# seongq/flowmse

Hardware: AMD Instinct MI355X
Metric: enhanced spectrogram-frames/sec at N=5 solver steps (higher is better)
Workload: dtype f32; 1 GPU; BASELINE config[1]: batch=8 synthetic complex spectrograms [8,1,256,256] per GPU, N=5 euler steps (5 NFE), NCSN++ (65.6M params, synthetic weights), precision mode fp32; global_batch=8, frames=256, solver_steps=5, parallelism=dp1 (per-utterance, final RCCL gather only), launch_mode=eager launches of the per-shape launch list (the library's default), hip_graph_launches=0, finite_output_checked=True

## Files before the change

flowmse_amd/csrc/common.h:

```cpp
#pragma once
#include <hip/hip_runtime.h>
#include <stdint.h>

namespace flowse {

enum { OK = 0, ERR_ARG = 1, ERR_HIP = 2, ERR_STATE = 3, ERR_SHAPE = 4 };

void set_error(const char* fmt, ...);
int hip_fail(hipError_t e, const char* what, const char* file, int line);

#define FLOWSE_HIP(call)                                                        \
    do {                                                                        \
        hipError_t _e = (call);                                                 \
        if (_e != hipSuccess) return ::flowse::hip_fail(_e, #call, __FILE__, __LINE__); \
    } while (0)

#define FLOWSE_LAUNCH_CHECK()                                                   \
    do {                                                                        \
        hipError_t _e = hipGetLastError();                                      \
        if (_e != hipSuccess) return ::flowse::hip_fail(_e, "kernel launch", __FILE__, __LINE__); \
    } while (0)

enum { DT_F32 = 0, DT_BF16 = 1, DT_F16 = 2 };
struct bf16_t { unsigned short v; };
// ... 61 lines not shown
    }
    static __device__ __forceinline__ float4 rnd4(float4 v) {
        return make_float4((float)(_Float16)v.x, (float)(_Float16)v.y, (float)(_Float16)v.z, (float)(_Float16)v.w);
    }
    static __device__ __forceinline__ float ld1(const f16_t* p) { return (float)__builtin_bit_cast(_Float16, p->v); }
    static __device__ __forceinline__ void st1(f16_t* p, float v) {
        const _Float16 x = (_Float16)v;
        p->v = __builtin_bit_cast(unsigned short, x);
    }
};
template <class ST> struct Vec16 { static constexpr int N = 16 / (int)sizeof(ST); };
template <class ST>
__device__ __forceinline__ void ld16(const ST* p, float* v) {
    if constexpr (sizeof(ST) == 4) {
        const float4 t = *reinterpret_cast<const float4*>(p);
        v[0] = t.x; v[1] = t.y; v[2] = t.z; v[3] = t.w;
    } else {
        const uint4 t = *reinterpret_cast<const uint4*>(p);
        const unsigned w[4] = {t.x, t.y, t.z, t.w};
#pragma unroll
        for (int i = 0; i < 4; ++i) {
            if constexpr (St<ST>::dt == DT_BF16) {
                v[2 * i] = __uint_as_float(w[i] << 16);
                v[2 * i + 1] = __uint_as_float(w[i] & 0xffff0000u);
            } else {
                v[2 * i] = (float)__builtin_bit_cast(_Float16, (unsigned short)(w[i] & 0xffffu));
                v[2 * i + 1] = (float)__builtin_bit_cast(_Float16, (unsigned short)(w[i] >> 16));
            }
        }
    }
}
template <class ST>
__device__ __forceinline__ void st16_round(ST* p, float* v) {
    if constexpr (sizeof(ST) == 4) {
        *reinterpret_cast<float4*>(p) = make_float4(v[0], v[1], v[2], v[3]);
    } else {
        unsigned w[4];
#pragma unroll
        for (int i = 0; i < 4; ++i) {
            if constexpr (St<ST>::dt == DT_BF16) {
                w[i] = St<bf16_t>::pack2(v[2 * i], v[2 * i + 1]);
                v[2 * i] = __uint_as_float(w[i] << 16);
                v[2 * i + 1] = __uint_as_float(w[i] & 0xffff0000u);
            } else {
                const _Float16 a = (_Float16)v[2 * i], b = (_Float16)v[2 * i + 1];
                w[i] = (unsigned)__builtin_bit_cast(unsigned short, a) | ((unsigned)__builtin_bit_cast(unsigned short, b) << 16);
                v[2 * i] = (float)a;
                v[2 * i + 1] = (float)b;
            }
        }
        *reinterpret_cast<uint4*>(p) = make_uint4(w[0], w[1], w[2], w[3]);
    }
}
#define FLOWSE_DT_SWITCH(dt, ST, ...)                                          \
    switch (dt) {                                                              \
        case ::flowse::DT_F32: { using ST = float; __VA_ARGS__; } break;       \
        case ::flowse::DT_BF16: { using ST = ::flowse::bf16_t; __VA_ARGS__; } break; \
        default: { using ST = ::flowse::f16_t; __VA_ARGS__; } break;           \
    }

struct GnParams {
    const float* mean;
    const float* scale;
    const float* beta;
};

struct Stat4 {
    float4 p, s1, s2;
    int n;
    __device__ __forceinline__ void init() {
        n = 0;
        p = s1 = s2 = make_float4(0.f, 0.f, 0.f, 0.f);
    }
    __device__ __forceinline__ void add(const float4& v) {
        if (n == 0) p = v;
        const float dx = v.x - p.x, dy = v.y - p.y, dz = v.z - p.z, dw = v.w - p.w;
        s1.x += dx; s1.y += dy; s1.z += dz; s1.w += dw;
        s2.x = fmaf(dx, dx, s2.x); s2.y = fmaf(dy, dy, s2.y); s2.z = fmaf(dz, dz, s2.z); s2.w = fmaf(dw, dw, s2.w);
        ++n;
    }
    __device__ __forceinline__ void finish(float* out8) const {
        const float inv = n > 0 ? 1.f / (float)n : 0.f;
        const float a[4] = {s1.x, s1.y, s1.z, s1.w}, q[4] = {s2.x, s2.y, s2.z, s2.w}, pv[4] = {p.x, p.y, p.z, p.w};
#pragma unroll
        for (int j = 0; j < 4; ++j) {
            out8[j] = pv[j] + a[j] * inv;
            out8[4 + j] = fmaxf(q[j] - a[j] * a[j] * inv, 0.f);
        }
    }
};
__device__ __forceinline__ void chan_merge4(float& nA, float* acc8, float nB, const float* in8) {
    if (nB <= 0.f) return;
    const float n = nA + nB, w = nB / n;
#pragma unroll
    for (int j = 0; j < 4; ++j) {
        const float d = in8[j] - acc8[j];
        acc8[j] += d * w;
        acc8[4 + j] += in8[4 + j] + d * d * nA * w;
    }
    nA = n;
}

struct ConvArgs {
    const float* in1;
    const float* in2;
    int C1, C2;
    const float* w;
    const float* bias;
    const float* bias2;
    int bias2_stride;
    const float* res;
    float* out;
    int B, H, W, Cout;
    int taps;
    float scale;
    int ksplit = 1;
    float* partial = nullptr;
    const float* partial2 = nullptr;
    int ksplit2 = 0;
    const float* bias_x = nullptr;
    float* stats = nullptr;
    int stats_nblk = 0;
    GnParams gn = {nullptr, nullptr, nullptr};
    int gn_silu = 0;
    const void* wq = nullptr;
    int terms = 0;
    int wq_f16 = 0;
    const void* wfrag = nullptr;
    const void* sc1 = nullptr;
    const void* sc2 = nullptr;
    int SC1 = 0, SC2 = 0;
    const void* wfrag_sc = nullptr;
    const float* wino = nullptr;
    const float* wino2 = nullptr;
    const float* wsm = nullptr;
    const float* wsm16 = nullptr;
    int in_dt = DT_F32, out_dt = DT_F32;
};
int conv16_ksplit(int B, int H, int W, int Cin, int Cout, int taps);
bool conv16_uses_halo(int B, int H, int W, int C1, int C2, int Cout, int taps);
void pc16_set_channel_blocks(int mode);
bool conv16_uses_pc(int B, int H, int W, int C1, int C2, int Cout, int taps);
int conv16_stats_blocks(int B, int H, int W, int Cin, int Cout, int taps);
int launch_convert(const void* src, int src_dt, void* dst, int dst_dt, int64_t n, hipStream_t s);
int launch_f43_weights(const float* w_packed, int Cout, int Cin, float* out, hipStream_t s);
int launch_pc16_weights(const void* w16, int Cout, int Cin, void* dst, hipStream_t s, int taps = 9);
bool conv16_smallm_ok(int B, int H, int W, int C1, int C2, int Cout, int taps);
int conv16_smallm_stats_blocks(int B, int H, int W);
inline int64_t conv_wino_numel(int Cout, int Cin) { return (int64_t)Cout * 18 * Cin; }
int launch_w2d_weights(const float* w_packed, int Cout, int Cin, float* out, hipStream_t s);
inline int64_t conv_w2d_numel(int Cout, int Cin) { return (int64_t)Cout * 24 * Cin; }
bool conv_w2d_shape_ok(int B, int H, int W, int C1, int C2, int Cout, int taps);
bool conv_supports_w2d(int B, int H, int W, int C1, int C2, int Cout, int taps);
bool conv_smallm_ok(int B, int H, int W, int C1, int C2, int Cout, int taps);
int launch_smallm_weights(const float* w_packed, int Cout, int taps, int Cin, float* out, hipStream_t s, bool tile16 = false);
bool conv_smallm_tile16(int B, int H, int W);
int conv_smallm_stats_blocks(int B, int H, int W);
bool conv1x1_stream_ok(int B, int H, int W, int C1, int C2, int Cout, int taps);
int conv1x1_stream_stats_blocks(int B, int H, int W);
bool conv_w2d_enabled();
bool conv_supports_wino(int B, int H, int W, int C1, int C2, int Cout, int taps);
bool conv_f43_wide(int B, int H, int W, int Cout);
void pack_conv_bf16(const float* w, int Cout, int Cin, int terms, uint16_t* dst, bool f16 = false);
inline int64_t conv_bf16_numel(int Cout, int Cin, int terms) { return (int64_t)Cout * 9 * Cin * (terms == 1 ? 1 : 2); }
bool conv_supports_bf16(int B, int H, int W, int C1, int C2, int Cout, int taps);
bool conv_supports_fused_gn(int B, int H, int W, int C1, int C2, int Cout, int taps);
bool conv_supports_head4(int B, int H, int W, int C1, int C2, int Cout, int taps);
int conv_fused_stats_blocks(int B, int H, int W, int Cin, int Cout, int taps);
int launch_conv(const ConvArgs& a, hipStream_t s, bool with_reduce = true);
int launch_splitk_reduce(const ConvArgs& a, hipStream_t s);
void conv_note_route(const char* a, const char* b = "", const char* c = "");
const char* conv_last_route();
bool conv_reduce_gn_ok(int B, int HW, int Cout);
int launch_splitk_reduce_gn(const ConvArgs& a, const float* gamma, const float* beta, float eps, int silu, int apply,
                            float* gn_mean, float* gn_scale, hipStream_t s);
int conv_ksplit(int B, int H, int W, int Cin, int Cout, int taps);
int conv_splitk_stats_group(int HW);
bool conv_splitk_is_wino(int B, int H, int W, int Cin, int Cout, int taps);
bool conv_cin4_uses_mfma(int B, int H, int W, int Cout, int taps);
int conv_cin4_stats_blocks(int B, int H, int W, int Cout);

int launch_conv_cin4(const ConvArgs& a, hipStream_t s);

int gn_partial_blocks(int HW, int C);
int gn_pixels_per_block(int HW, int nblk);
int launch_gn_stats(const void* in1, int C1, const void* in2, int C2, int B, int HW,
                    float* partial , int nblk, hipStream_t s, int dt = DT_F32);
int launch_gn_finalize(const float* partial1, int nblk1, int C1, const float* partial2, int nblk2, int C2, int B,
                       int HW, int G, const float* gamma, float eps, float* mean ,
                       float* scale , hipStream_t s);

int launch_gn_finalize_apply(const void* in1, const float* partial1, int nblk1, int C1, const void* in2,
                             const float* partial2, int nblk2, int C2, int B, int HW, int G, const float* gamma,
                             const float* beta, float eps, int silu, void* out, hipStream_t s, int in_dt = DT_F32,
                             int out_dt = DT_F32);
int launch_gn_apply(const void* in1, int C1, const void* in2, int C2, int B, int HW,
                    GnParams gn, int silu, void* out, hipStream_t s, int in_dt = DT_F32, int out_dt = DT_F32);

int launch_fir_down(const void* in, int B, int H, int W, int C, GnParams gn, int silu, void* out,
                    hipStream_t s, void* out2 = nullptr, int dt = DT_F32);
int launch_fir_up(const void* in, int B, int H, int W, int C, GnParams gn, int silu, const void* add,
                  void* out, hipStream_t s, void* out2 = nullptr, int dt = DT_F32);
int launch_upfirdn2d_nchw(const float* in, const float* kernel, int planes, int in_h, int in_w, int kh,
                          int kw, int up_x, int up_y, int down_x, int down_y, int pad_x0, int pad_x1,
                          int pad_y0, int pad_y1, float* out, int out_h, int out_w, hipStream_t s);

int launch_attention(const void* qkv, int B, int L, int C, void* out, hipStream_t s, int dt = DT_F32);

struct CallBlock {
    const float* x;
    const float* y;
    const float* t;
    float* out;
    int mode;
    float dt;
    const float* x0 = nullptr;
    const float* acc_in = nullptr;
    float* acc_out = nullptr;
    float a = 0.f, b = 0.f;
};
int launch_set_call(CallBlock* d_cb, const CallBlock& value, hipStream_t s);
int launch_fill_times(float* d_ts, const float* ts, int N, int B, hipStream_t s);
int launch_pack_input(const float* x_c64, const float* y_c64, int B, int F, int T, float* out4, hipStream_t s,
                      const CallBlock* cb = nullptr);
int launch_gfp(const float* t, const float* Wf, int B, int E, float* out, hipStream_t s, const CallBlock* cb = nullptr);
int launch_linear(const float* in, int B, int K, const float* W, const float* bias, int R, int act,
                  float* out, int out_stride, hipStream_t s);
int launch_head(const float* pyr4, const float* t, const float* Wout , const float* bout ,
                int B, int F, int T, int mode, const float* x_c64, float dt, float* out_c64, hipStream_t s,
                const CallBlock* cb = nullptr);
int launch_stft_compress(const float* sig, int B, int L, float scale_in, float* out_c64, int T, int Tpad, float factor,
                         float exponent, hipStream_t s);
int launch_istft_decompress(const float* spec_c64, int B, int T, int Tpad, float factor, float exponent, float* out,
                            int Lout, float scale_out, hipStream_t s);
int launch_stft_compress_chunks(const float* sig, int L, float scale_in, float* out_c64, int K, int Tc, int hop,
                                float factor, float exponent, hipStream_t s);
int launch_istft_decompress_chunks(const float* chunks_c64, int K, int Tc, int hop, float factor, float exponent,
                                   float* out, int Lout, float scale_out, hipStream_t s);
int launch_axpy(const float* y, const float* z, float sigma, int64_t n, float* out, hipStream_t s);
int launch_keyed_noise(const float* y, const uint64_t* keys, const int32_t* frame0, uint64_t seed, float sigma, float* out,
                       int B, int F, int T, hipStream_t s);

}
```

flowmse_amd/csrc/conv_w2d.hip:

```cpp
#include "conv_common.h"

#ifdef FLOWSE_MEASURE_W2D
namespace flowse { __device__ unsigned long long g_w2d_ts[256 * 64]; }
extern "C" int flowse_debug_w2d_ts(unsigned long long* host, int n) {
    return hipMemcpyFromSymbol(host, HIP_SYMBOL(flowse::g_w2d_ts), (size_t)n * 8) == hipSuccess ? 0 : 1;
}
#ifdef FLOWSE_MEASURE_W2D_WAVES
#define W2_TS(K) if ((threadIdx.x & 63) == 0 && blockIdx.x < 256 && (K) >= 4 && ((K) - 4) % 3 == 0 && ((K) - 4) / 3 < 8) \
        flowse::g_w2d_ts[blockIdx.x * 64 + (threadIdx.x >> 6) * 8 + ((K) - 4) / 3] = __builtin_amdgcn_s_memrealtime();
#else
#define W2_TS(K) if (threadIdx.x == 0 && blockIdx.x < 256 && (K) < 64) flowse::g_w2d_ts[blockIdx.x * 64 + (K)] = __builtin_amdgcn_s_memrealtime();
#endif
#else
#define W2_TS(K)
#endif

namespace flowse {

constexpr int W2_HROW = 18 * LDS_ROW + 8;
constexpr int W2_HBUF = 18 * W2_HROW;
constexpr int W2_XDEST = 4 * 3 * 256;

struct W2Tile {
    int y0, x0;
    unsigned hin;
    unsigned woff;
};

template <int CH, int NJ>
__device__ __forceinline__ void w2d_out(f32x16 (&acc)[3][NJ], float* X, int b, int y0, int x0, int n0) {
    const ConvArgs* ap = (const ConvArgs*)__builtin_amdgcn_kernarg_segment_ptr();
    asm volatile("" : "+s"(ap));
    const ConvArgs& a = *ap;
    const int tid = threadIdx.x;
    int lane = tid & 63;
    asm volatile("" : "+v"(lane));
    const int wave = __builtin_amdgcn_readfirstlane(tid >> 6);
    const int hq = wave & 3;
    const int jD = wave >> 2, gD = wave & 3;
    const bool dest = jD < NJ;
    const int li = lane & 31, kh = lane >> 5;
    const int W = a.W, Cout = a.Cout;
    const int ch0 = n0 + jD * 32;
    const int pl = lane >> 3, cq = lane & 7;
    const bool has_res = a.res != nullptr;
    const int64_t pix0 = ((int64_t)b * a.H + y0 + 4 * gD) * W + x0;
    const float* resb = a.res + pix0 * Cout + ch0 + cq * 4;
    float* outb = a.out + pix0 * Cout + ch0 + cq * 4;
    int roff[8];
#pragma unroll
    for (int i = 0; i < 8; ++i) {
        const int pp = i * 8 + pl;
        roff[i] = ((pp >> 4) * W + (pp & 15)) * Cout;
    }
    float4 rres[8];
    if (has_res && dest) {
#pragma unroll
        for (int i = 0; i < 8; ++i) rres[i] = *reinterpret_cast<const float4*>(resb + roff[i]);
    }
    float* Xd = X + wave * W2_XDEST;
    auto give = [&]() {
#pragma unroll
        for (int D = 0; D < 4 * NJ; ++D) {
            const int jd = D >> 2, gd = D & 3;
            float4 v0, v1, v2;
            float* e0 = &v0.x; float* e1 = &v1.x; float* e2 = &v2.x;
#pragma unroll
            for (int e = 0; e < 4; ++e) {
                const int r = 4 * gd + e;
                const float s12 = acc[1][jd][r] + acc[2][jd][r];
                if (CH == 0) {
                    e0[e] = acc[0][jd][r] + s12;
                    e1[e] = acc[1][jd][r] - acc[2][jd][r];
                    e2[e] = s12;
                } else {
                    e0[e] = s12;
                    e1[e] = acc[1][jd][r] - acc[2][jd][r];
                    e2[e] = acc[0][jd][r];
                }
            }
            float* dst = X + D * W2_XDEST + (hq * 3) * 256 + lane * 4;
            *reinterpret_cast<float4*>(dst) = v0;
            *reinterpret_cast<float4*>(dst + 256) = v1;
            *reinterpret_cast<float4*>(dst + 512) = v2;
        }
    };
    auto take = [&](float (&S)[2][3][4]) {
#pragma unroll
        for (int s = 0; s < 4; ++s) {
#pragma unroll
            for (int c = 0; c < 3; ++c) {
                const float4 t = *reinterpret_cast<const float4*>(Xd + (s * 3 + c) * 256 + lane * 4);
                const float* q = &t.x;
#pragma unroll
                for (int e = 0; e < 4; ++e) {
                    if (s == 0) S[0][c][e] = q[e];
                    if (s == 1) { S[0][c][e] += q[e]; S[1][c][e] = q[e]; }
                    if (s == 2) { S[0][c][e] += q[e]; S[1][c][e] -= q[e]; }
                    if (s == 3) S[1][c][e] -= q[e];
                }
            }
        }
    };
    float SA[2][3][4], SB[2][3][4];
    if (CH == 0) give();
    __syncthreads();
    if (dest) take(SA);
    __syncthreads();
    if (CH == 1) give();
    __syncthreads();
    if (!dest) return;
    float4 bq = make_float4(0.f, 0.f, 0.f, 0.f), bq2 = bq;
    if (a.bias) bq = *reinterpret_cast<const float4*>(a.bias + ch0 + cq * 4);
    if (a.bias2) bq2 = *reinterpret_cast<const float4*>(a.bias2 + (int64_t)b * a.bias2_stride + ch0 + cq * 4);
    take(SB);
    float* T = Xd;
    __builtin_amdgcn_wave_barrier();
#pragma unroll
    for (int x = 0; x < 2; ++x)
#pragma unroll
        for (int e = 0; e < 4; ++e) {
            const float A = SA[x][0][e], Bv = SA[x][1][e], Cv = SA[x][2][e];
            const float D = SB[x][0][e], E = SB[x][1][e], Fv = SB[x][2][e];
            const float o0 = A + D, o1 = fmaf(2.f, E, Bv), o2 = fmaf(4.f, D, Cv), o3 = fmaf(8.f, E, Bv) + Fv;
            const int col = 2 * (e + 4 * kh) + x;
            T[(0 * 16 + col) * 32 + li] = o0;
            T[(1 * 16 + col) * 32 + li] = o1;
            T[(2 * 16 + col) * 32 + li] = o2;
            T[(3 * 16 + col) * 32 + li] = o3;
        }
    __builtin_amdgcn_wave_barrier();
    bq.x += bq2.x; bq.y += bq2.y; bq.z += bq2.z; bq.w += bq2.w;
    const float scale = a.scale;
    float4 piv = make_float4(0.f, 0.f, 0.f, 0.f), s1 = piv, s2 = piv;
#pragma unroll
    for (int i = 0; i < 8; ++i) {
        const int pp = i * 8 + pl;
        float4 v = *reinterpret_cast<const float4*>(T + pp * 32 + cq * 4);
        v.x += bq.x; v.y += bq.y; v.z += bq.z; v.w += bq.w;
        if (has_res) { v.x += rres[i].x; v.y += rres[i].y; v.z += rres[i].z; v.w += rres[i].w; }
        v.x *= scale; v.y *= scale; v.z *= scale; v.w *= scale;
        *reinterpret_cast<float4*>(outb + roff[i]) = v;
        if (i == 0) piv = v;
        const float dx = v.x - piv.x, dy = v.y - piv.y, dz = v.z - piv.z, dw = v.w - piv.w;
        s1.x += dx; s1.y += dy; s1.z += dz; s1.w += dw;
        s2.x = fmaf(dx, dx, s2.x); s2.y = fmaf(dy, dy, s2.y); s2.z = fmaf(dz, dz, s2.z); s2.w = fmaf(dw, dw, s2.w);
    }
    if (!a.stats) return;
    float mean[4] = {piv.x + s1.x * 0.125f, piv.y + s1.y * 0.125f, piv.z + s1.z * 0.125f, piv.w + s1.w * 0.125f};
    float m2[4] = {fmaxf(s2.x - s1.x * s1.x * 0.125f, 0.f), fmaxf(s2.y - s1.y * s1.y * 0.125f, 0.f),
                   fmaxf(s2.z - s1.z * s1.z * 0.125f, 0.f), fmaxf(s2.w - s1.w * s1.w * 0.125f, 0.f)};
    float cnt = 8.f;
#pragma unroll
    for (int off = 8; off < 64; off <<= 1) {
#pragma unroll
        for (int j = 0; j < 4; ++j) {
            const float mo = __shfl_xor(mean[j], off), qo = __shfl_xor(m2[j], off);
            const float d = mo - mean[j];
            m2[j] = m2[j] + qo + d * d * (0.5f * cnt);
            mean[j] = 0.5f * (mean[j] + mo);
        }
        cnt *= 2.f;
    }
    if (pl == 0) {
        const int strip = ((y0 >> 2) + gD) * (W >> 4) + (x0 >> 4);
        float* dst = a.stats + (((int64_t)b * a.stats_nblk + strip) * Cout + ch0 + cq * 4) * 2;
        *reinterpret_cast<float4*>(dst) = make_float4(mean[0], m2[0], mean[1], m2[1]);
        *reinterpret_cast<float4*>(dst + 4) = make_float4(mean[2], m2[2], mean[3], m2[3]);
    }
}

template <int GN, int CH, int NJ>
__device__ __forceinline__ void conv3x3_w2d_body(const ConvArgs& a, float* smem, int tpb) {
    constexpr int BN = 32 * NJ;
    constexpr int H_LOADS = 6;
    float* Hs = smem;

    const int tid = threadIdx.x;
    W2_TS(0)
    const int H = a.H, W = a.W, HW = H * W;
    const int C1 = a.C1, C2 = a.C2, Cin = C1 + C2;
    const int n_ntiles = a.Cout / BN;
    const int bid = xcd_remap(blockIdx.x, gridDim.x);
    const int mg = bid / n_ntiles;
    const int nt = bid - mg * n_ntiles;
    const int tiles_x = W >> 4, tiles_img = tiles_x * (H >> 4);
    const int n0 = nt * BN;
    const int wave = __builtin_amdgcn_readfirstlane(tid >> 6);
    const int col4 = tid & 7, slot = tid >> 3;
    const bool s_on = slot < 54;
    const int s_hx = slot >= 36 ? 2 : slot >= 18 ? 1 : 0, s_hy = slot - 18 * s_hx;
    const unsigned s_pix = (unsigned)(s_hy * W + s_hx);
    const int s_lds = s_hy * W2_HROW + s_hx * LDS_ROW + 4 * (col4 ^ ((s_hy >> 2) & 1));
    int s_st = s_lds + W2_HBUF;
    int dflip = W2_HBUF;
    const int bsmp = (mg * tpb) / tiles_img;
    const int b = bsmp;
    const int64_t sbase = (int64_t)bsmp * HW - W - 1;
    const int spix = HW + 2 * W + 2;
    const __amdgpu_buffer_rsrc_t rsrc1 =
        __builtin_amdgcn_make_buffer_rsrc(const_cast<float*>(a.in1 + sbase * C1), 0, spix * C1 * 4, 0x00020000);
    const __amdgpu_buffer_rsrc_t rsrc2 = __builtin_amdgcn_make_buffer_rsrc(
        const_cast<float*>(C2 ? a.in2 + sbase * C2 : a.in1), 0, C2 ? spix * C2 * 4 : 0, 0x00020000);
    auto make_tile = [&](int mt) {
        W2Tile t;
        const int tt = mt - bsmp * tiles_img;
        int ty, tx;
        if ((tiles_x & 3) == 0) {
            const int per_strip = 4 * (H >> 4);
            const int strip = tt / per_strip, w = tt - strip * per_strip;
            ty = w >> 2;
            tx = strip * 4 + (w & 3);
        } else {
            ty = tt / tiles_x;
            tx = tt - ty * tiles_x;
        }
        t.y0 = ty * 16;
        t.x0 = tx * 16;
        const bool rowin = s_on && (unsigned)(t.y0 - 1 + s_hy) < (unsigned)H;
        t.hin = 0;
#pragma unroll
        for (int q = 0; q < H_LOADS; ++q)
            t.hin |= (rowin && (unsigned)(t.x0 - 1 + s_hx + 3 * q) < (unsigned)W) ? (1u << q) : 0u;
        t.woff = (unsigned)(t.y0 * W + t.x0);
        return t;
    };
    const W2Tile first = make_tile(mg * tpb);
    int cur_y0 = first.y0, cur_x0 = first.x0;
    const __amdgpu_buffer_rsrc_t rsrcw =
        __builtin_amdgcn_make_buffer_rsrc(const_cast<float*>(a.wino2), 0, a.Cout * 24 * Cin * 4, 0x00020000);

    u32x4 rh[3];
    float4 g_mu, g_sc, g_be;
    unsigned st_hin = first.hin;

    auto hload = [&](const W2Tile& t, int chunk, int Q) -> u32x4 {
        const int c0 = chunk * KC;
        const bool second = c0 >= C1;
        const unsigned cs = (unsigned)(second ? C2 : C1);
        const unsigned soff = ((t.woff + 3u * (unsigned)Q) * cs + (unsigned)(second ? c0 - C1 : c0)) * 4u;
        const unsigned off = ((t.hin >> Q) & 1u) ? (s_pix * cs + (unsigned)col4 * 4u) * 4u : OOB;
        return second ? __builtin_amdgcn_raw_buffer_load_b128(rsrc2, off, soff, 0)
                      : __builtin_amdgcn_raw_buffer_load_b128(rsrc1, off, soff, 0);
    };
    auto gparams = [&](int chunk, unsigned hin) {
        if (GN) {
            const int cg = chunk * KC + col4 * 4;
            const float rowf = (hin >> 1) & 1u ? 1.f : 0.f;
            g_mu = *reinterpret_cast<const float4*>(a.gn.mean + (int64_t)b * Cin + cg);
            g_sc = *reinterpret_cast<const float4*>(a.gn.scale + (int64_t)b * Cin + cg);
            g_be = *reinterpret_cast<const float4*>(a.gn.beta + cg);
            g_sc.x *= rowf; g_sc.y *= rowf; g_sc.z *= rowf; g_sc.w *= rowf;
            g_be.x *= rowf; g_be.y *= rowf; g_be.z *= rowf; g_be.w *= rowf;
        }
    };
    auto gloadH = [&](const W2Tile& t, int chunk, int h) {
#pragma unroll
        for (int q = 0; q < 3; ++q) rh[q] = hload(t, chunk, 3 * h + q);
        if (h == 0) {
            gparams(chunk, t.hin);
            st_hin = t.hin;
        }
    };
    auto xform1 = [&](int Q) {
        if (GN) rh[Q % 3] = gn_quad<GN>(rh[Q % 3], g_mu, g_sc, g_be, (Q == 0 || Q == 5) ? ((st_hin >> Q) & 1u) != 0 : true);
    };
    auto lstoreH = [&](int h) {
        float* Hb = Hs + s_st + 9 * h * LDS_ROW;
        if (s_on) {
#pragma unroll
            for (int q = 0; q < 3; ++q) *reinterpret_cast<u32x4*>(Hb + 3 * q * LDS_ROW) = rh[q];
        }
    };

    const int lane = tid & 63;
    const int hq = wave & 3;
    const int li = lane & 31, kh = lane >> 5;
    const int ur = li >> 3, uc = li & 7;
    const int ca = hq == 0 ? 0 : hq == 2 ? 2 : 1, cb = hq == 2 ? 1 : hq == 3 ? 3 : 2;
    f32x2 sg2 = {hq == 1 ? 1.f : -1.f, hq == 1 ? 1.f : -1.f};
    asm volatile("" : "+v"(sg2));
    const int base = (4 * ur + CH) * W2_HROW + 2 * uc * LDS_ROW;
    const int k0 = 4 * (kh ^ (ur & 1)), k1 = 4 * (kh ^ (ur & 1) ^ 1);
    int aA0 = base + ca * LDS_ROW + k0, aA1 = base + ca * LDS_ROW + k1;
    int aB0 = base + cb * LDS_ROW + k0, aB1 = base + cb * LDS_ROW + k1;

    const int nchunks = Cin / KC;
    const unsigned wslice = (unsigned)((n0 >> 5) * 4 + hq) * (unsigned)nchunks;
    const unsigned wvo = (unsigned)lane * 16u + (unsigned)CH * 3u * 4096u;
    unsigned wvoc[3] = {wvo, wvo + 4096u, wvo + 8192u};
    asm volatile("" : "+v"(wvoc[0]), "+v"(wvoc[1]), "+v"(wvoc[2]));
    const unsigned wj = 4u * (unsigned)nchunks * 24576u;

    f32x16 acc[3][NJ];

    {
        u32x4 t[H_LOADS];
#pragma unroll
        for (int q = 0; q < H_LOADS; ++q) t[q] = hload(first, 0, q);
        gparams(0, first.hin);
#pragma unroll
        for (int q = 0; q < H_LOADS; ++q) {
            if (GN) t[q] = gn_quad<GN>(t[q], g_mu, g_sc, g_be, (q == 0 || q == 5) ? ((first.hin >> q) & 1u) != 0 : true);
            if (s_on) *reinterpret_cast<u32x4*>(Hs + s_lds + 3 * q * LDS_ROW) = t[q];
        }
    }
    __syncthreads();
    W2_TS(1)

#define W2_FENCE __builtin_amdgcn_sched_barrier(0);
#define W2_RD(BASE0, BASE1, R, J) \
    (*reinterpret_cast<const float4*>(Hs + ((CH + (R)) >= 4 ? (BASE1) : (BASE0)) + (R) * W2_HROW + (J) * 8))
#define W2_BLOAD(C, JT, J, WB, BF)                                                                                   \
    {                                                                                                                \
        const u32x4 t = __builtin_amdgcn_raw_buffer_load_b128(rsrcw, wvoc[C] + (J) * 1024, WB[JT], 0);               \
        BF[C][JT] = make_float4(__uint_as_float(t.x), __uint_as_float(t.y), __uint_as_float(t.z),                    \
                                __uint_as_float(t.w));                                                               \
    }
#define W2_H2(Q, H) (*reinterpret_cast<f32x2*>(&(Q).x + 2 * (H)))
#define W2_COMB(D, T, R, TR)                                                                                             \
    {                                                                                                                \
        W2_H2(D[R], 0) = __builtin_elementwise_fma(sg2, W2_H2(T[TR], 0), W2_H2(D[R], 0));                            \
        W2_H2(D[R], 1) = __builtin_elementwise_fma(sg2, W2_H2(T[TR], 1), W2_H2(D[R], 1));                            \
    }
#define W2_WXA_H(D, h)                                                                                               \
    {                                                                                                                \
        const f32x2 c4 = {4.f, 4.f}, cm5 = {-5.f, -5.f};                                                             \
        const f32x2 r0 = W2_H2(D[0], h), r2 = W2_H2(D[2], h), r4 = W2_H2(D[4], h);                                   \
        const f32x2 v = __builtin_elementwise_fma(c4, r0, __builtin_elementwise_fma(cm5, r2, r4));                   \
        if (CH == 0) W2_H2(D[0], h) = v;                                                                             \
        else W2_H2(D[4], h) = v;                                                                                     \
    }
#define W2_WXB_H(D, h)                                                                                               \
    {                                                                                                                \
        const f32x2 c4 = {4.f, 4.f}, cm4 = {-4.f, -4.f}, c2 = {2.f, 2.f}, cm2 = {-2.f, -2.f};                        \
        const f32x2 r0 = W2_H2(D[0], h), r1 = W2_H2(D[1], h), r2 = W2_H2(D[2], h), r3 = W2_H2(D[3], h),              \
                    r4 = W2_H2(D[4], h);                                                                             \
        if (CH == 0) {                                                                                               \
            W2_H2(D[1], h) = __builtin_elementwise_fma(cm4, r1 + r2, r3 + r4);                                       \
            W2_H2(D[2], h) = __builtin_elementwise_fma(c4, r1 - r2, r4 - r3);                                        \
        } else {                                                                                                     \
            W2_H2(D[1], h) = __builtin_elementwise_fma(c2, r2 - r0, r3 - r1);                                        \
            W2_H2(D[2], h) = __builtin_elementwise_fma(cm2, r2 - r0, r3 - r1);                                       \
        }                                                                                                            \
    }
#define W2_WXA(D) { W2_WXA_H(D, 0) W2_WXA_H(D, 1) }
#define W2_WXB(D) { W2_WXB_H(D, 0) W2_WXB_H(D, 1) }
#define W2_MF(V, c, K)                                                                                               \
    _Pragma("unroll") for (int j = 0; j < NJ; ++j)                                                                   \
        acc[c][j] = __builtin_amdgcn_mfma_f32_32x32x2f32(V[((c) == 0 && CH == 1) ? 4 : (c)].K, bF[c][j].K, acc[c][j], 0, 0, 0); \
    W2_FENCE
#define W2_BL(C, NJB, WB) _Pragma("unroll") for (int j = 0; j < NJ; ++j) W2_BLOAD(C, j, NJB, WB, bF)
#define W2_PHASE(V, DN, NJB, WB, SX)                                                                                 \
    W2_MF(V, 0, x) DN[0] = W2_RD(aA0, aA1, 0, NJB); tN[0] = W2_RD(aB0, aB1, 0, NJB);                                 \
                   DN[1] = W2_RD(aA0, aA1, 1, NJB); tN[1] = W2_RD(aB0, aB1, 1, NJB); W2_FENCE                        \
    W2_MF(V, 0, y) DN[2] = W2_RD(aA0, aA1, 2, NJB); tN[2] = W2_RD(aB0, aB1, 2, NJB); W2_COMB(DN, tN, 0, 0) W2_FENCE  \
    W2_MF(V, 0, z) DN[3] = W2_RD(aA0, aA1, 3, NJB); tN[0] = W2_RD(aB0, aB1, 3, NJB); W2_COMB(DN, tN, 1, 1) W2_FENCE  \
    W2_MF(V, 0, w) DN[4] = W2_RD(aA0, aA1, 4, NJB); tN[1] = W2_RD(aB0, aB1, 4, NJB); W2_COMB(DN, tN, 2, 2) W2_FENCE  \
    W2_MF(V, 1, x) W2_BL(0, NJB, WB) W2_COMB(DN, tN, 3, 0) W2_FENCE                                                  \
    W2_MF(V, 1, y) W2_COMB(DN, tN, 4, 1) W2_WXA_H(DN, 0) W2_FENCE                                                    \
    W2_MF(V, 1, z) W2_WXA_H(DN, 1) W2_WXB_H(DN, 0) W2_FENCE                                                          \
    W2_MF(V, 1, w) W2_WXB_H(DN, 1) W2_FENCE                                                                          \
    W2_MF(V, 2, x) W2_BL(1, NJB, WB) W2_FENCE                                                                        \
    W2_MF(V, 2, y) SX W2_FENCE                                                                                       \
    W2_MF(V, 2, z)                                                                                                   \
    W2_MF(V, 2, w) W2_BL(2, NJB, WB) W2_FENCE

    float4 dA[5], dB[5], tN[3], bF[3][NJ];
    auto start_issue = [&]() {
#pragma unroll
        for (int r = 0; r < 5; ++r) dA[r] = W2_RD(aA0, aA1, r, 0);
#pragma unroll
        for (int r = 0; r < 3; ++r) tN[r] = W2_RD(aB0, aB1, r, 0);
        const unsigned wb[2] = {wslice * 24576u, wslice * 24576u + wj};
#pragma unroll
        for (int c = 0; c < 3; ++c)
#pragma unroll
            for (int j = 0; j < NJ; ++j) W2_BLOAD(c, j, 0, wb, bF)
    };
    auto start_finish = [&]() {
#pragma unroll
        for (int r = 0; r < 3; ++r) W2_COMB(dA, tN, r, r)
#pragma unroll
        for (int r = 3; r < 5; ++r) tN[r - 3] = W2_RD(aB0, aB1, r, 0);
#pragma unroll
        for (int r = 3; r < 5; ++r) W2_COMB(dA, tN, r, r - 3)
        W2_WXA(dA) W2_WXB(dA)
    };
    const int nslots = tpb * nchunks;
    int sg_t = 0, sg_c = 0;
    W2Tile stg = first;
    auto stage_advance = [&]() {
        if (++sg_c == nchunks) {
            sg_c = 0;
            ++sg_t;
            if (sg_t < tpb) stg = make_tile(mg * tpb + sg_t);
        }
        if (sg_t >= tpb) {
            sg_t = tpb;
            sg_c = nchunks - 1;
        }
    };
    stage_advance();
    gloadH(stg, sg_c, 0);
    start_issue();
    start_finish();
    int ti = 0, chunk = 0;
#pragma unroll
    for (int c = 0; c < 3; ++c)
#pragma unroll
        for (int j = 0; j < NJ; ++j)
#pragma unroll
            for (int r = 0; r < 16; ++r) acc[c][j][r] = 0.f;
    for (int slot = 0; slot < nslots; ++slot) {
        const bool last = chunk + 1 == nchunks;
        const unsigned wb[2] = {(wslice + (unsigned)chunk) * 24576u, (wslice + (unsigned)chunk) * 24576u + wj};
        const unsigned wbn0 = last ? wslice * 24576u : wb[0] + 24576u;
        const unsigned wbn[2] = {wbn0, wbn0 + wj};
        W2_PHASE(dA, dB, 1, wb, { xform1(0); xform1(1); })
        W2_PHASE(dB, dA, 2, wb, { xform1(2); lstoreH(0); gloadH(stg, sg_c, 1); })
        W2_PHASE(dA, dB, 3, wb, { xform1(3); xform1(4); })
        xform1(5);
        lstoreH(1);
        W2_TS(4 + 3 * slot)
        __syncthreads();
        W2_TS(5 + 3 * slot)
        aA0 += dflip; aA1 += dflip; aB0 += dflip; aB1 += dflip;
        s_st -= dflip;
        dflip = -dflip;
        asm volatile("" : "+v"(aA0), "+v"(aA1), "+v"(aB0), "+v"(aB1), "+v"(s_st));
        stage_advance();
        W2_PHASE(dB, dA, 0, wbn, { gloadH(stg, sg_c, 0); })
        W2_TS(6 + 3 * slot)
        if (last) {
            const bool more = ti + 1 < tpb;
            w2d_out<CH, NJ>(acc, smem + W2_HBUF, b, cur_y0, cur_x0, n0);
            W2_TS(2 + (ti & 1))
            if (!more) return;
            __syncthreads();
            start_issue();
            start_finish();
            {
                const W2Tile nx = make_tile(mg * tpb + ti + 1);
                cur_y0 = nx.y0;
                cur_x0 = nx.x0;
            }
#pragma unroll
            for (int c = 0; c < 3; ++c)
#pragma unroll
                for (int j = 0; j < NJ; ++j)
#pragma unroll
                    for (int r = 0; r < 16; ++r) acc[c][j][r] = 0.f;
            ++ti;
            chunk = 0;
        } else {
            ++chunk;
        }
    }
#undef W2_FENCE
#undef W2_RD
#undef W2_BLOAD
#undef W2_H2
#undef W2_COMB
#undef W2_WXA
#undef W2_WXB
#undef W2_WXA_H
#undef W2_WXB_H
#undef W2_MF
#undef W2_BL
#undef W2_PHASE
}

template <int GN, int NJ>
__global__ __launch_bounds__(512, 2) void conv3x3_w2d_kernel(ConvArgs a, int tpb) {
    extern __shared__ __attribute__((aligned(16))) float smem[];
    if (__builtin_amdgcn_readfirstlane(threadIdx.x >> 8)) conv3x3_w2d_body<GN, 1, NJ>(a, smem, tpb);
    else conv3x3_w2d_body<GN, 0, NJ>(a, smem, tpb);
}

__global__ __launch_bounds__(256) void w2d_weights_kernel(const float* __restrict__ w, int Cout, int Cin,
                                                          float* __restrict__ out) {
    const int64_t idx = (int64_t)blockIdx.x * 256 + threadIdx.x;
    if (idx >= (int64_t)Cout * Cin) return;
    const int ci = (int)(idx % Cin);
    const int64_t n = idx / Cin;
    float U[6][3];
#pragma unroll
    for (int kx = 0; kx < 3; ++kx) {
        const float g0 = w[(n * 9 + 0 + kx) * Cin + ci], g1 = w[(n * 9 + 3 + kx) * Cin + ci],
                    g2 = w[(n * 9 + 6 + kx) * Cin + ci];
        const float s02 = g0 + g2;
        U[0][kx] = 0.25f * g0;
        U[1][kx] = (s02 + g1) * (-1.f / 6.f);
        U[2][kx] = (s02 - g1) * (-1.f / 6.f);
        const float t = fmaf(g0, 1.f / 24.f, g2 * (1.f / 6.f)), h = g1 * (1.f / 12.f);
        U[3][kx] = g2;
        U[4][kx] = t + h;
        U[5][kx] = t - h;
    }
    const int nchunks = Cin >> 5;
    const int chunk = ci >> 5, j = (ci >> 3) & 3, kh = (ci >> 2) & 1, e = ci & 3;
    const int lane = kh * 32 + (int)(n & 31);
#pragma unroll
// ... 79 lines not shown
```

flowmse_amd/csrc/model_api.hip:

```cpp
#include "model.h"

namespace flowse {

static void drop_graph(Plan* p) {
    if (p->exec) (void)hipGraphExecDestroy(p->exec);
    if (p->graph) (void)hipGraphDestroy(p->graph);
    p->exec = nullptr;
    p->graph = nullptr;
    p->eager_runs = 0;
}

static void clear_plans(flowse_model* m) {
    for (auto& kv : m->plans) drop_graph(&kv.second);
    m->plans.clear();
    m->block_plans.clear();
}

static int check_device(const flowse_model* m) {
    int dev = 0;
    FLOWSE_HIP(hipGetDevice(&dev));
    if (m->wt->device >= 0 && dev != m->wt->device) {
        set_error("model handle is bound to HIP device %d but device %d is current (reload the weights on the new "
                  "device, or hipSetDevice back)", m->wt->device, dev);
        return ERR_STATE;
// ... 945 lines not shown

int flowse_upfirdn2d(const float* input, const float* kernel, int planes, int in_h, int in_w, int kh, int kw, int up_x,
                     int up_y, int down_x, int down_y, int pad_x0, int pad_x1, int pad_y0, int pad_y1, float* out,
                     int out_h, int out_w, void* stream) {
    if (!input || !kernel || !out || pad_x0 < 0 || pad_x1 < 0 || pad_y0 < 0 || pad_y1 < 0) {
        set_error("flowse_upfirdn2d: bad argument (null pointer or negative pad)");
        return ERR_ARG;
    }
    return launch_upfirdn2d_nchw(input, kernel, planes, in_h, in_w, kh, kw, up_x, up_y, down_x, down_y, pad_x0, pad_x1,
                                 pad_y0, pad_y1, out, out_h, out_w, static_cast<hipStream_t>(stream));
}

int64_t flowse_op_conv2d_scratch_floats(int B, int H, int W, int Cin, int Cout, int taps) {
    if (conv_smallm_ok(B, H, W, Cin, 0, Cout, taps) || conv1x1_stream_ok(B, H, W, Cin, 0, Cout, taps))
        return (int64_t)Cout * taps * Cin;
    const int ks = conv_ksplit(B, H, W, Cin, Cout, taps);
    return ks > 1 ? (int64_t)ks * B * H * W * Cout : 0;
}

int flowse_op_conv2d(const float* in1, int C1, const float* in2, int C2, const float* w, const float* bias,
                     const float* bias2, int bias2_stride, const float* res, float* out, int B, int H, int W, int Cout,
                     int taps, float scale, float* splitk_scratch, void* stream) {
    if (!in1 || !w || !out) {
        set_error("flowse_op_conv2d: null argument");
        return ERR_ARG;
    }
    ConvArgs c;
    c.in1 = in1; c.in2 = in2; c.C1 = C1; c.C2 = in2 ? C2 : 0;
    c.w = w; c.bias = bias; c.bias2 = bias2; c.bias2_stride = bias2_stride; c.res = res; c.out = out;
    c.B = B; c.H = H; c.W = W; c.Cout = Cout; c.taps = taps; c.scale = scale;
    hipStream_t s = static_cast<hipStream_t>(stream);
    if (C1 == 4 && !in2) return launch_conv_cin4(c, s);
    if (splitk_scratch && conv1x1_stream_ok(B, H, W, c.C1, c.C2, Cout, taps)) {
        const int rc = launch_smallm_weights(w, Cout, taps, c.C1 + c.C2, splitk_scratch, s, false);
        if (rc != OK) return rc;
        c.wsm = splitk_scratch;
    } else if (splitk_scratch && conv_smallm_ok(B, H, W, c.C1, c.C2, Cout, taps)) {
        const bool t16 = conv_smallm_tile16(B, H, W);
        const int rc = launch_smallm_weights(w, Cout, taps, c.C1 + c.C2, splitk_scratch, s, t16);
        if (rc != OK) return rc;
        c.wsm = splitk_scratch;
        c.wsm16 = t16 ? splitk_scratch : nullptr;
    } else if (splitk_scratch) {
        c.ksplit = conv_ksplit(B, H, W, c.C1 + c.C2, Cout, taps);
        c.partial = c.ksplit > 1 ? splitk_scratch : nullptr;
    }
    return launch_conv(c, s);
}

int64_t flowse_op_group_norm_scratch_floats(int B, int HW, int C) {
    const int nblk = gn_partial_blocks(HW, C);
    return (int64_t)B * nblk * C * 2 + 2 * (int64_t)B * C;
}

int flowse_op_group_norm(const float* in1, int C1, const float* in2, int C2, const float* gamma, const float* beta,
                         float eps, int silu, float* out, int B, int H, int W, float* scratch, void* stream) {
    if (!in1 || !gamma || !beta || !out || !scratch) {
        set_error("flowse_op_group_norm: null argument");
        return ERR_ARG;
    }
    hipStream_t s = static_cast<hipStream_t>(stream);
    if (!in2) C2 = 0;
    const int C = C1 + C2, HW = H * W;
    const int G = std::min(C / 4, 32);
    const int nblk = gn_partial_blocks(HW, C);
    float* part = scratch;
    float* mean = scratch + (int64_t)B * nblk * C * 2;
    float* scl = mean + (int64_t)B * C;
    int rc = launch_gn_stats(in1, C1, in2, C2, B, HW, part, nblk, s);
    if (rc != OK) return rc;
    rc = launch_gn_finalize(part, nblk, C, nullptr, 0, 0, B, HW, G, gamma, eps, mean, scl, s);
    if (rc != OK) return rc;
    GnParams p{mean, scl, beta};
    return launch_gn_apply(in1, C1, in2, C2, B, HW, p, silu, out, s);
}

int flowse_op_conv3x3_gn(const float* in1, int C1, const float* in2, int C2, const float* gamma, const float* beta,
                         float eps, int silu, const float* w, const float* bias, const float* bias2, int bias2_stride,
                         const float* res, float* out, int B, int H, int W, int Cout, float scale, float* scratch,
                         void* stream) {
    if (!in1 || !gamma || !beta || !w || !out || !scratch) {
        set_error("flowse_op_conv3x3_gn: null argument");
        return ERR_ARG;
    }
    if (!in2) C2 = 0;
    if (!conv_supports_fused_gn(B, H, W, C1, C2, Cout, 9)) {
        set_error("flowse_op_conv3x3_gn: shape B=%d H=%d W=%d C=%d+%d Cout=%d not covered by the halo kernel", B, H, W,
                  C1, C2, Cout);
        return ERR_SHAPE;
    }
    hipStream_t s = static_cast<hipStream_t>(stream);
    const int C = C1 + C2, HW = H * W;
    const int G = std::min(C / 4, 32);
    const int nblk = gn_partial_blocks(HW, C);
    float* part = scratch;
    float* mean = scratch + (int64_t)B * nblk * C * 2;
    float* scl = mean + (int64_t)B * C;
    int rc = launch_gn_stats(in1, C1, in2, C2, B, HW, part, nblk, s);
    if (rc != OK) return rc;
    rc = launch_gn_finalize(part, nblk, C, nullptr, 0, 0, B, HW, G, gamma, eps, mean, scl, s);
    if (rc != OK) return rc;
    ConvArgs c;
    c.in1 = in1; c.in2 = in2; c.C1 = C1; c.C2 = C2;
    c.w = w; c.bias = bias; c.bias2 = bias2; c.bias2_stride = bias2_stride; c.res = res; c.out = out;
    c.B = B; c.H = H; c.W = W; c.Cout = Cout; c.taps = 9; c.scale = scale;
    c.gn = GnParams{mean, scl, beta};
    c.gn_silu = silu;
    return launch_conv(c, s);
}

static int op_conv3x3_winograd(const float* in1, int C1, const float* in2, int C2, const float* gamma,
                               const float* beta, float eps, int silu, const float* w, const float* bias,
                               const float* bias2, int bias2_stride, const float* res, float* out, int B, int H, int W,
                               int Cout, float scale, float* scratch, void* stream, bool two_d = false) {
    if (!in1 || !w || !out || !scratch || (gamma && !beta)) {
        set_error("flowse_op_conv3x3_f43: null argument");
        return ERR_ARG;
    }
    if (!in2) C2 = 0;
    if (two_d ? !conv_w2d_shape_ok(B, H, W, C1, C2, Cout, 9) : !conv_supports_wino(B, H, W, C1, C2, Cout, 9)) {
        set_error("flowse_op_conv3x3_%s: shape B=%d H=%d W=%d C=%d+%d Cout=%d not covered by the Winograd kernel",
                  two_d ? "w2d" : "f43", B, H, W, C1, C2, Cout);
        return ERR_SHAPE;
    }
    hipStream_t s = static_cast<hipStream_t>(stream);
    const int C = C1 + C2, HW = H * W;
    float* wf = scratch + flowse_op_group_norm_scratch_floats(B, HW, C);
    int rc = two_d ? launch_w2d_weights(w, Cout, C, wf, s) : launch_f43_weights(w, Cout, C, wf, s);
    if (rc != OK) return rc;
    ConvArgs c;
    c.in1 = in1; c.in2 = in2; c.C1 = C1; c.C2 = C2;
    c.w = w; c.bias = bias; c.bias2 = bias2; c.bias2_stride = bias2_stride; c.res = res; c.out = out;
    c.B = B; c.H = H; c.W = W; c.Cout = Cout; c.taps = 9; c.scale = scale;
    if (two_d) c.wino2 = wf;
    else c.wino = wf;
    const int ks = two_d ? 1 : conv_ksplit(B, H, W, C, Cout, 9);
    if (ks > 1) {
        c.ksplit = ks;
        c.partial = wf + conv_wino_numel(Cout, C);
    }
    if (gamma) {
        const int G = std::min(C / 4, 32);
        const int nblk = gn_partial_blocks(HW, C);
        float* part = scratch;
        float* mean = scratch + (int64_t)B * nblk * C * 2;
        float* scl = mean + (int64_t)B * C;
        rc = launch_gn_stats(in1, C1, in2, C2, B, HW, part, nblk, s);
        if (rc != OK) return rc;
        rc = launch_gn_finalize(part, nblk, C, nullptr, 0, 0, B, HW, G, gamma, eps, mean, scl, s);
        if (rc != OK) return rc;
        c.gn = GnParams{mean, scl, beta};
        c.gn_silu = silu;
    }
    return launch_conv(c, s);
}

int64_t flowse_op_conv3x3_f43_scratch_floats(int B, int H, int W, int C, int Cout) {
    const int ks = conv_ksplit(B, H, W, C, Cout, 9);
    return flowse_op_group_norm_scratch_floats(B, H * W, C) + conv_wino_numel(Cout, C) +
           (ks > 1 ? (int64_t)ks * B * H * W * Cout : 0);
}

int64_t flowse_op_conv3x3_w2d_scratch_floats(int B, int H, int W, int C, int Cout) {
    return flowse_op_group_norm_scratch_floats(B, H * W, C) + conv_w2d_numel(Cout, C);
}

int flowse_op_conv3x3_w2d(const float* in1, int C1, const float* in2, int C2, const float* gamma, const float* beta,
                          float eps, int silu, const float* w, const float* bias, const float* bias2, int bias2_stride,
                          const float* res, float* out, int B, int H, int W, int Cout, float scale, float* scratch,
                          void* stream) {
    return op_conv3x3_winograd(in1, C1, in2, C2, gamma, beta, eps, silu, w, bias, bias2, bias2_stride, res, out, B, H,
                               W, Cout, scale, scratch, stream, true);
}

int flowse_op_conv3x3_f43(const float* in1, int C1, const float* in2, int C2, const float* gamma, const float* beta,
                          float eps, int silu, const float* w, const float* bias, const float* bias2, int bias2_stride,
                          const float* res, float* out, int B, int H, int W, int Cout, float scale, float* scratch,
                          void* stream) {
    return op_conv3x3_winograd(in1, C1, in2, C2, gamma, beta, eps, silu, w, bias, bias2, bias2_stride, res, out, B, H,
                               W, Cout, scale, scratch, stream);
}

static int op_conv2d_16(const float* in1, int C1, const float* in2, int C2, const float* w, const float* bias,
                        const float* bias2, int bias2_stride, const float* res, const float* gn_mean, const float* gn_scale,
                        const float* gn_beta, int silu, float* out, int out_f32, int B, int H, int W, int Cout, int taps,
                        float scale, int dt, void* scratch, int64_t scratch_bytes, void* stream) {
    if (!in1 || !w || !out || !scratch || (dt != DT_BF16 && dt != DT_F16) || (taps != 1 && taps != 9)) {
        set_error("flowse_op_conv2d_16: bad argument");
        return ERR_ARG;
    }
    if (!in2) C2 = 0;
    hipStream_t s = static_cast<hipStream_t>(stream);
    const int64_t M = (int64_t)B * H * W, C = C1 + C2;
    const bool halo = !out_f32 && conv16_uses_halo(B, H, W, C1, C2, Cout, taps);
    const bool head = Cout == 4 && taps == 9 && !in2 && conv_supports_head4(B, H, W, C1, 0, Cout, taps);
    const int ks = (halo || head) ? 1 : conv16_ksplit(B, H, W, (int)C, Cout, taps);
    const int64_t nw = ((int64_t)Cout * taps * C + 3) & ~(int64_t)3;
    auto up = [](int64_t b) { return (b + 255) & ~(int64_t)255; };
    const int64_t need = up(2 * M * C1) + up(2 * M * C2) + 2 * up(2 * nw) + 2 * up(2 * M * Cout) +
                         (ks > 1 ? up(4 * (int64_t)ks * M * Cout) : 0);
    if (scratch_bytes < need) {
        set_error("flowse_op_conv2d_16: scratch needs %lld bytes", (long long)need);
        return ERR_ARG;
    }
    if (gn_mean && !halo && !head) {
        set_error("flowse_op_conv2d_16: fused GroupNorm input only on LDS-halo shapes");
        return ERR_SHAPE;
    }
    char* p = static_cast<char*>(scratch);
    auto take = [&](int64_t bytes) { char* q = p; p += (bytes + 255) & ~(int64_t)255; return q; };
    void* a1 = take(2 * M * C1);
    void* a2 = C2 ? take(2 * M * C2) : nullptr;
    void* wq = take(2 * nw);
    const bool frag = (taps == 9 && conv16_uses_pc(B, H, W, C1, C2, Cout, taps)) || conv16_smallm_ok(B, H, W, C1, C2, Cout, taps);
    void* wfrag = frag ? take(2 * nw) : nullptr;
    const bool direct = head || out_f32;
    void* r16 = res && !direct ? take(2 * M * Cout) : nullptr;
    void* o16 = direct ? nullptr : take(2 * M * Cout);
    float* part = ks > 1 ? reinterpret_cast<float*>(take(4 * (int64_t)ks * M * Cout)) : nullptr;
    if ((size_t)(p - static_cast<char*>(scratch)) > (size_t)scratch_bytes) {
        set_error("flowse_op_conv2d_16: scratch too small");
        return ERR_ARG;
    }
    int rc = launch_convert(in1, DT_F32, a1, dt, M * C1, s);
    if (rc == OK && C2) rc = launch_convert(in2, DT_F32, a2, dt, M * C2, s);
    if (rc == OK) rc = launch_convert(w, DT_F32, wq, dt, nw, s);
    if (rc == OK && frag) rc = launch_pc16_weights(wq, Cout, (int)C, wfrag, s, taps);
    if (rc == OK && r16) rc = launch_convert(res, DT_F32, r16, dt, M * Cout, s);
    if (rc != OK) return rc;
    ConvArgs c;
    c.in1 = static_cast<const float*>(a1); c.in2 = static_cast<const float*>(a2); c.C1 = C1; c.C2 = C2;
    c.w = w; c.bias = bias; c.bias2 = bias2; c.bias2_stride = bias2 ? bias2_stride : 0;
    c.res = static_cast<const float*>(r16); c.out = static_cast<float*>(o16);
    c.B = B; c.H = H; c.W = W; c.Cout = Cout; c.taps = taps; c.scale = scale;
    c.ksplit = ks; c.partial = part;
    c.wq = wq; c.terms = 1; c.wq_f16 = dt == DT_F16 ? 1 : 0;
    c.wfrag = wfrag;
    c.in_dt = dt; c.out_dt = dt;
    if (gn_mean) {
        c.gn = GnParams{gn_mean, gn_scale, gn_beta};
        c.gn_silu = silu;
    }
    if (direct) {
        c.res = res;
        c.out = out;
        c.out_dt = DT_F32;
    }
    rc = launch_conv(c, s);
    if (rc != OK || direct) return rc;
    return launch_convert(o16, dt, out, DT_F32, M * Cout, s);
}

int flowse_op_conv2d_16(const float* in1, int C1, const float* in2, int C2, const float* w, const float* bias,
                        const float* res, const float* gn_mean, const float* gn_scale, const float* gn_beta, int silu,
                        float* out, int B, int H, int W, int Cout, int taps, float scale, int dt, void* scratch,
                        int64_t scratch_bytes, void* stream) {
    return op_conv2d_16(in1, C1, in2, C2, w, bias, nullptr, 0, res, gn_mean, gn_scale, gn_beta, silu, out, 0, B, H, W, Cout,
                        taps, scale, dt, scratch, scratch_bytes, stream);
}

int flowse_op_conv2d_16_ex(const float* in1, int C1, const float* in2, int C2, const float* w, const float* bias,
                           const float* bias2, int bias2_stride, const float* res, const float* gn_mean,
                           const float* gn_scale, const float* gn_beta, int silu, float* out, int out_f32, int B, int H,
                           int W, int Cout, int taps, float scale, int dt, void* scratch, int64_t scratch_bytes,
                           void* stream) {
    if (bias2 && (bias2_stride < Cout || (bias2_stride & 3))) {
        set_error("flowse_op_conv2d_16_ex: bias2_stride must be a multiple of 4 and at least Cout");
        return ERR_ARG;
    }
    return op_conv2d_16(in1, C1, in2, C2, w, bias, bias2, bias2_stride, res, gn_mean, gn_scale, gn_beta, silu, out,
                        out_f32 != 0, B, H, W, Cout, taps, scale, dt, scratch, scratch_bytes, stream);
}

const char* flowse_op_last_conv_route(void) { return conv_last_route(); }

int flowse_op_resblock_tail_16(const float* h, int C, const float* gn_mean, const float* gn_scale, const float* gn_beta,
                               int silu, const float* w1, const float* b1, const float* x1, int XC1, const float* x2,
                               int XC2, const float* w2, const float* b2, float* out, int B, int H, int W, int Cout,
                               float scale, int dt, void* scratch, int64_t scratch_bytes, void* stream) {
    if (!h || !w1 || !x1 || !w2 || !out || !scratch || (dt != DT_BF16 && dt != DT_F16)) {
        set_error("flowse_op_resblock_tail_16: bad argument");
        return ERR_ARG;
    }
    if (!x2) XC2 = 0;
    if (!conv16_uses_pc(B, H, W, C, 0, Cout, 9)) {
        set_error("flowse_op_resblock_tail_16: only shapes conv3x3_pc16_kernel takes (H, W multiples of 16, C %% 32 == 0, "
                  "Cout %% 128 == 0, >= 64 tile x channel-block items)");
        return ERR_SHAPE;
    }
    hipStream_t s = static_cast<hipStream_t>(stream);
    const int64_t M = (int64_t)B * H * W, XC = (int64_t)XC1 + XC2;
    const int64_t nw1 = ((int64_t)Cout * 9 * C + 3) & ~(int64_t)3, nw2 = ((int64_t)Cout * XC + 3) & ~(int64_t)3;
    auto up = [](int64_t b) { return (b + 255) & ~(int64_t)255; };
    const int64_t need = up(2 * M * C) + up(2 * M * XC1) + up(2 * M * XC2) + 2 * up(2 * nw1) + 2 * up(2 * nw2) + up(2 * M * Cout);
    if (scratch_bytes < need) {
        set_error("flowse_op_resblock_tail_16: scratch needs %lld bytes", (long long)need);
        return ERR_ARG;
    }
    char* p = static_cast<char*>(scratch);
    auto take = [&](int64_t bytes) { char* q = p; p += (bytes + 255) & ~(int64_t)255; return q; };
    void* h16 = take(2 * M * C);
    void* a1 = take(2 * M * XC1);
    void* a2 = XC2 ? take(2 * M * XC2) : nullptr;
    void* wq1 = take(2 * nw1);
    void* wf1 = take(2 * nw1);
    void* wq2 = take(2 * nw2);
    void* wf2 = take(2 * nw2);
// ... 70 lines not shown
```

Measured before the change: 22580 frames/s.

## Transpose W2D MFMA operands to drop LDS output transpose in epilogue

```diff
diff --git a/flowmse_amd/csrc/common.h b/flowmse_amd/csrc/common.h
--- a/flowmse_amd/csrc/common.h
+++ b/flowmse_amd/csrc/common.h
@@ -237,6 +237,7 @@
 inline int64_t conv_w2d_numel(int Cout, int Cin) { return (int64_t)Cout * 24 * Cin; }
 bool conv_w2d_shape_ok(int B, int H, int W, int C1, int C2, int Cout, int taps);
 bool conv_supports_w2d(int B, int H, int W, int C1, int C2, int Cout, int taps);
+int launch_w2d(const ConvArgs& a, hipStream_t s);
 bool conv_smallm_ok(int B, int H, int W, int C1, int C2, int Cout, int taps);
 int launch_smallm_weights(const float* w_packed, int Cout, int taps, int Cin, float* out, hipStream_t s, bool tile16 = false);
 bool conv_smallm_tile16(int B, int H, int W);
diff --git a/flowmse_amd/csrc/conv_w2d.hip b/flowmse_amd/csrc/conv_w2d.hip
--- a/flowmse_amd/csrc/conv_w2d.hip
+++ b/flowmse_amd/csrc/conv_w2d.hip
@@ -40,49 +40,49 @@
     const int jD = wave >> 2, gD = wave & 3;
     const bool dest = jD < NJ;
     const int li = lane & 31, kh = lane >> 5;
+    const int ur = li >> 3, uc = li & 7;
     const int W = a.W, Cout = a.Cout;
     const int ch0 = n0 + jD * 32;
-    const int pl = lane >> 3, cq = lane & 7;
+    const int ucD = lane >> 3, cq = lane & 7;
     const bool has_res = a.res != nullptr;
-    const int64_t pix0 = ((int64_t)b * a.H + y0 + 4 * gD) * W + x0;
+    const int64_t pix0 = ((int64_t)b * a.H + y0 + 4 * gD) * W + x0 + 2 * ucD;
     const float* resb = a.res + pix0 * Cout + ch0 + cq * 4;
     float* outb = a.out + pix0 * Cout + ch0 + cq * 4;
-    int roff[8];
-#pragma unroll
-    for (int i = 0; i < 8; ++i) {
-        const int pp = i * 8 + pl;
-        roff[i] = ((pp >> 4) * W + (pp & 15)) * Cout;
-    }
+    auto poff = [&](int i) { return ((i >> 1) * W + (i & 1)) * Cout; };
     float4 rres[8];
     if (has_res && dest) {
 #pragma unroll
-        for (int i = 0; i < 8; ++i) rres[i] = *reinterpret_cast<const float4*>(resb + roff[i]);
-    }
-    float* Xd = X + wave * W2_XDEST;
+        for (int i = 0; i < 8; ++i) rres[i] = *reinterpret_cast<const float4*>(resb + poff(i));
+    }
+    const int gpos = (uc * 8 + (kh ^ uc)) ^ ((ur & 1) << 3);
+    float* Xs = X + ur * W2_XDEST + (hq * 3) * 256;
+    const float* Xd = X + wave * W2_XDEST + 4 * ((lane ^ ucD) ^ ((gD & 1) << 3));
     auto give = [&]() {
 #pragma unroll
-        for (int D = 0; D < 4 * NJ; ++D) {
-            const int jd = D >> 2, gd = D & 3;
-            float4 v0, v1, v2;
-            float* e0 = &v0.x; float* e1 = &v1.x; float* e2 = &v2.x;
-#pragma unroll
-            for (int e = 0; e < 4; ++e) {
-                const int r = 4 * gd + e;
-                const float s12 = acc[1][jd][r] + acc[2][jd][r];
-                if (CH == 0) {
-                    e0[e] = acc[0][jd][r] + s12;
-                    e1[e] = acc[1][jd][r] - acc[2][jd][r];
-                    e2[e] = s12;
-                } else {
-                    e0[e] = s12;
-                    e1[e] = acc[1][jd][r] - acc[2][jd][r];
-                    e2[e] = acc[0][jd][r];
+        for (int jd = 0; jd < NJ; ++jd) {
+#pragma unroll
+            for (int q = 0; q < 4; ++q) {
+                float4 v0, v1, v2;
+                float* e0 = &v0.x; float* e1 = &v1.x; float* e2 = &v2.x;
+#pragma unroll
+                for (int e = 0; e < 4; ++e) {
+                    const int r = 4 * q + e;
+                    const float s12 = acc[1][jd][r] + acc[2][jd][r];
+                    if (CH == 0) {
+                        e0[e] = acc[0][jd][r] + s12;
+                        e1[e] = acc[1][jd][r] - acc[2][jd][r];
+                        e2[e] = s12;
+                    } else {
+                        e0[e] = s12;
+                        e1[e] = acc[1][jd][r] - acc[2][jd][r];
+                        e2[e] = acc[0][jd][r];
+                    }
                 }
+                float* dst = Xs + jd * 4 * W2_XDEST + 4 * (gpos ^ (2 * q));
+                *reinterpret_cast<float4*>(dst) = v0;
+                *reinterpret_cast<float4*>(dst + 256) = v1;
+                *reinterpret_cast<float4*>(dst + 512) = v2;
             }
-            float* dst = X + D * W2_XDEST + (hq * 3) * 256 + lane * 4;
-            *reinterpret_cast<float4*>(dst) = v0;
-            *reinterpret_cast<float4*>(dst + 256) = v1;
-            *reinterpret_cast<float4*>(dst + 512) = v2;
         }
     };
     auto take = [&](float (&S)[2][3][4]) {
@@ -90,7 +90,7 @@
         for (int s = 0; s < 4; ++s) {
 #pragma unroll
             for (int c = 0; c < 3; ++c) {
-                const float4 t = *reinterpret_cast<const float4*>(Xd + (s * 3 + c) * 256 + lane * 4);
+                const float4 t = *reinterpret_cast<const float4*>(Xd + (s * 3 + c) * 256);
                 const float* q = &t.x;
 #pragma unroll
                 for (int e = 0; e < 4; ++e) {
@@ -114,33 +114,28 @@
     if (a.bias) bq = *reinterpret_cast<const float4*>(a.bias + ch0 + cq * 4);
     if (a.bias2) bq2 = *reinterpret_cast<const float4*>(a.bias2 + (int64_t)b * a.bias2_stride + ch0 + cq * 4);
     take(SB);
-    float* T = Xd;
-    __builtin_amdgcn_wave_barrier();
+    float o[4][2][4];
 #pragma unroll
     for (int x = 0; x < 2; ++x)
 #pragma unroll
         for (int e = 0; e < 4; ++e) {
             const float A = SA[x][0][e], Bv = SA[x][1][e], Cv = SA[x][2][e];
             const float D = SB[x][0][e], E = SB[x][1][e], Fv = SB[x][2][e];
-            const float o0 = A + D, o1 = fmaf(2.f, E, Bv), o2 = fmaf(4.f, D, Cv), o3 = fmaf(8.f, E, Bv) + Fv;
-            const int col = 2 * (e + 4 * kh) + x;
-            T[(0 * 16 + col) * 32 + li] = o0;
-            T[(1 * 16 + col) * 32 + li] = o1;
-            T[(2 * 16 + col) * 32 + li] = o2;
-            T[(3 * 16 + col) * 32 + li] = o3;
-        }
-    __builtin_amdgcn_wave_barrier();
+            o[0][x][e] = A + D;
+            o[1][x][e] = fmaf(2.f, E, Bv);
+            o[2][x][e] = fmaf(4.f, D, Cv);
+            o[3][x][e] = fmaf(8.f, E, Bv) + Fv;
+        }
     bq.x += bq2.x; bq.y += bq2.y; bq.z += bq2.z; bq.w += bq2.w;
     const float scale = a.scale;
     float4 piv = make_float4(0.f, 0.f, 0.f, 0.f), s1 = piv, s2 = piv;
 #pragma unroll
     for (int i = 0; i < 8; ++i) {
-        const int pp = i * 8 + pl;
-        float4 v = *reinterpret_cast<const float4*>(T + pp * 32 + cq * 4);
+        float4 v = make_float4(o[i >> 1][i & 1][0], o[i >> 1][i & 1][1], o[i >> 1][i & 1][2], o[i >> 1][i & 1][3]);
         v.x += bq.x; v.y += bq.y; v.z += bq.z; v.w += bq.w;
         if (has_res) { v.x += rres[i].x; v.y += rres[i].y; v.z += rres[i].z; v.w += rres[i].w; }
         v.x *= scale; v.y *= scale; v.z *= scale; v.w *= scale;
-        *reinterpret_cast<float4*>(outb + roff[i]) = v;
+        *reinterpret_cast<float4*>(outb + poff(i)) = v;
         if (i == 0) piv = v;
         const float dx = v.x - piv.x, dy = v.y - piv.y, dz = v.z - piv.z, dw = v.w - piv.w;
         s1.x += dx; s1.y += dy; s1.z += dz; s1.w += dw;
@@ -162,7 +157,7 @@
         }
         cnt *= 2.f;
     }
-    if (pl == 0) {
+    if (ucD == 0) {
         const int strip = ((y0 >> 2) + gD) * (W >> 4) + (x0 >> 4);
         float* dst = a.stats + (((int64_t)b * a.stats_nblk + strip) * Cout + ch0 + cq * 4) * 2;
         *reinterpret_cast<float4*>(dst) = make_float4(mean[0], m2[0], mean[1], m2[1]);
@@ -348,7 +343,7 @@
 #define W2_WXB(D) { W2_WXB_H(D, 0) W2_WXB_H(D, 1) }
 #define W2_MF(V, c, K)                                                                                               \
     _Pragma("unroll") for (int j = 0; j < NJ; ++j)                                                                   \
-        acc[c][j] = __builtin_amdgcn_mfma_f32_32x32x2f32(V[((c) == 0 && CH == 1) ? 4 : (c)].K, bF[c][j].K, acc[c][j], 0, 0, 0); \
+        acc[c][j] = __builtin_amdgcn_mfma_f32_32x32x2f32(bF[c][j].K, V[((c) == 0 && CH == 1) ? 4 : (c)].K, acc[c][j], 0, 0, 0); \
     W2_FENCE
 #define W2_BL(C, NJB, WB) _Pragma("unroll") for (int j = 0; j < NJ; ++j) W2_BLOAD(C, j, NJB, WB, bF)
 #define W2_PHASE(V, DN, NJB, WB, SX)                                                                                 \
diff --git a/flowmse_amd/csrc/model_api.hip b/flowmse_amd/csrc/model_api.hip
--- a/flowmse_amd/csrc/model_api.hip
+++ b/flowmse_amd/csrc/model_api.hip
@@ -1121,7 +1121,7 @@
         c.gn = GnParams{mean, scl, beta};
         c.gn_silu = silu;
     }
-    return launch_conv(c, s);
+    return two_d ? launch_w2d(c, s) : launch_conv(c, s);
 }
 
 int64_t flowse_op_conv3x3_f43_scratch_floats(int B, int H, int W, int C, int Cout) {
```

New measurement: 22940 frames/s, median of 6. 1.6% higher.
